# vitoplantamura/OnnxStream

Hardware: NVIDIA H100
Metric: SD1.5 UNet 512x512 bs=1 denoise steps/s (one UNet Model::run per step) (higher is better)
Workload: dtype f16

## Files before the change

### onnxstream_b200/csrc/attention_wgmma.cu

```cuda

#include "common.cuh"
#include "tc_ptx.cuh"
#include <cuda.h>
#include <cstdio>

namespace {

using namespace tcptx;

constexpr int BQ = 128;
constexpr int BKV = 128;
constexpr int KV_STAGES = 4;
constexpr int FA_THREADS = 384;
constexpr int FA_CONSUMERS = 256;
constexpr int FA_PRODUCER_REGS = 40, FA_CONSUMER_REGS = 232;

template <int NCH, int BK, int QKS, int KS = KV_STAGES, int PLANES = 1>
struct FaCfg {
    static_assert(QKS <= 4 * NCH && (BK == 32 || BK == 64 || BK == 128), "tile");
    static constexpr int Q_CHUNK = BQ * 128;
    static constexpr int KV_CHUNK = BK * 128;
    static constexpr int Q_PLANE = NCH * Q_CHUNK;
    static constexpr int KV_PLANE = NCH * KV_CHUNK;
    static constexpr int Q_BYTES = PLANES * Q_PLANE;
// ... 33 lines not shown
    return smem;
}

template <int KS, typename Load>
__device__ __forceinline__ void fa_produce_kv(uint64_t* kv_full, uint64_t* kv_empty, int n_kv, uint32_t tile_bytes, Load load)
{
    for (int j = 0; j < n_kv; j++) {
        const int st = j % KS;
        mbar_wait(&kv_empty[st], ((j / KS) & 1) ^ 1);
        if (elect_one()) {
            mbar_expect_tx(&kv_full[st], tile_bytes);
            load(st, j, &kv_full[st]);
        }
        __syncwarp();
    }
    osb_pdl_trigger_late();
}

template <int BK>
__device__ __forceinline__ float fa_row_max(const float (&s)[BK / 2], int h)
{
    float mt = -INFINITY;
#pragma unroll
    for (int c = 0; c < BK / 8; c++) mt = fmaxf(mt, fmaxf(s[4 * c + 2 * h], s[4 * c + 2 * h + 1]));
    mt = fmaxf(mt, __shfl_xor_sync(0xffffffffu, mt, 1));
    mt = fmaxf(mt, __shfl_xor_sync(0xffffffffu, mt, 2));
    return mt;
}

__device__ __forceinline__ float ex2_approx(float x)
{
// ... 110 lines not shown
#pragma unroll
            for (int h = 0; h < 2; h++) { o[ch][4 * c + 2 * h] *= alpha[h]; o[ch][4 * c + 2 * h + 1] *= alpha[h]; }
#pragma unroll
    for (int c = 0; c < BK / 8; c++)
#pragma unroll
        for (int h = 0; h < 2; h++) a[c >> 1][(c & 1) * 2 + h] = pack_half2(s[4 * c + 2 * h], s[4 * c + 2 * h + 1]);
}

template <int NCH, int BK, int QKS>
__global__ void __launch_bounds__(FA_THREADS, 1)
flash_attention_kernel(const __grid_constant__ CUtensorMap map_q, const __grid_constant__ CUtensorMap map_k, const __grid_constant__ CUtensorMap map_v,
                       const FaParams p)
{
    using C = FaCfg<NCH, BK, QKS>;
    constexpr int S = KV_STAGES;
    osb_pdl_trigger_entry();
    const int warp = threadIdx.x >> 5, lane = threadIdx.x & 31;
    const int head = blockIdx.y;
    const int q0 = blockIdx.x * BQ;
    const int n_kv = p.kv_tiles;
    uint8_t* smem = fa_prologue(&map_q, &map_k, &map_v, C::BARS, FA_CONSUMERS / 32, S);
    uint8_t* sQ = smem;
    uint8_t* sK = sQ + C::Q_BYTES;
    uint8_t* sV = sK + S * C::KV_BYTES;
    uint64_t* q_full = (uint64_t*)(smem + C::BARS);
    uint64_t* kv_full = q_full + 1;
    uint64_t* kv_empty = kv_full + S;

    if (warp < 4) {
        setmaxnreg_dec<FA_PRODUCER_REGS>();
        if (warp == 0) {
// ... 100 lines not shown
    const unsigned short* m = reinterpret_cast<const unsigned short*>(row) + col;
    if (col + 1 < Tk) {
        if (vec) return __ldg(reinterpret_cast<const unsigned int*>(m));
        return (uint32_t)__ldg(m) | ((uint32_t)__ldg(m + 1) << 16);
    }
    return col < Tk ? (uint32_t)__ldg(m) : 0u;
}

template <int NCH, int BK>
__global__ void __launch_bounds__(FA_THREADS, 1)
sdpa_flash_kernel(const __grid_constant__ CUtensorMap map_q, const __grid_constant__ CUtensorMap map_k, const __grid_constant__ CUtensorMap map_v,
                  const SdpaParams p)
{
    using C = FaCfg<NCH, BK, 4 * NCH>;
    constexpr float LOG2E = 1.4426950408889634f;
    osb_pdl_trigger_entry();
    const int warp = threadIdx.x >> 5, lane = threadIdx.x & 31;
    const int r0 = blockIdx.x * BQ, hk = blockIdx.y;
    const int n_kv = p.kv_tiles;
    uint8_t* smem = fa_prologue(&map_q, &map_k, &map_v, C::BARS, FA_CONSUMERS, KV_STAGES);
    uint8_t* sQ = smem;
    uint8_t* sK = sQ + C::Q_BYTES;
    uint8_t* sV = sK + KV_STAGES * C::KV_BYTES;
    uint64_t* q_full = (uint64_t*)(smem + C::BARS);
    uint64_t* kv_full = q_full + 1;
    uint64_t* kv_empty = kv_full + KV_STAGES;

    if (warp == 0) {
        if (elect_one()) {
            mbar_expect_tx(q_full, C::Q_BYTES);
#pragma unroll
// ... 152 lines not shown
    wgmma_fence();
#pragma unroll
    for (int kk = 0; kk < WD_BK / 16; kk++)
#pragma unroll
        for (int ch = 0; ch < WD_NV; ch++)
            wgmma_m64n64k16_f16_rs(o[ch], a[kk], vdesc + (uint64_t)((ch * WD_V_CHUNK + kk * 2048) >> 4), 1u);
    wgmma_commit();
}

template <bool KT>
__global__ void __launch_bounds__(WD_THREADS, 1)
flash_attention_wide_kernel(const __grid_constant__ CUtensorMap map_q, const __grid_constant__ CUtensorMap map_k,
                            const __grid_constant__ CUtensorMap map_v, const FaParams p)
{
    constexpr int KS = WD_K_STAGES, VS = WD_V_STAGES;
    osb_pdl_trigger_entry();
    const int warp = threadIdx.x >> 5, lane = threadIdx.x & 31;
    const int n_slices = (p.d + 64 * WD_NV - 1) / (64 * WD_NV);
    const int col0 = (blockIdx.x % n_slices) * (64 * WD_NV);
    const int q0 = (blockIdx.x / n_slices) * WD_BQ;
    const int head = blockIdx.y;
    const int n_dch = (p.d + 63) >> 6;
    uint8_t* smem = fa_prologue(&map_q, &map_k, &map_v, WD_BARS, WD_CONSUMERS / 32, KS, VS);
    uint8_t* sQ = smem;
    uint8_t* sK = sQ + WD_DCH * WD_Q_CHUNK;
    uint8_t* sV = sK + KS * WD_K_CHUNK;
    uint64_t* q_full = (uint64_t*)(smem + WD_BARS);
    uint64_t* k_full = q_full + 1;
    uint64_t* k_empty = k_full + KS;
    uint64_t* v_full = k_empty + KS;
    uint64_t* v_empty = v_full + VS;
// ... 17 lines not shown
                        mbar_expect_tx(&k_full[st], WD_K_CHUNK);
                        if (KT) tma_load_3d(sK + st * WD_K_CHUNK, &map_k, &k_full[st], j * WD_BK, 64 * c, head);
                        else tma_load_3d(sK + st * WD_K_CHUNK, &map_k, &k_full[st], 64 * c, j * WD_BK, head);
                    }
                    __syncwarp();
                }
                const int sv = j % VS;
                mbar_wait(&v_empty[sv], ((j / VS) & 1) ^ 1);
                if (elect_one()) {
                    mbar_expect_tx(&v_full[sv], n_vch * WD_V_CHUNK);
                    for (int ch = 0; ch < n_vch; ch++)
                        tma_load_3d(sV + sv * WD_V_BYTES + ch * WD_V_CHUNK, &map_v, &v_full[sv], col0 + 64 * ch, j * WD_BK, head);
                }
                __syncwarp();
            }
            osb_pdl_trigger_late();
        }
    } else {
        setmaxnreg_inc<WD_CONSUMER_REGS>();
        const int r = (warp & 3) * 16 + (lane >> 2);
        const int cq = 2 * (lane & 3);
        const uint64_t qdesc0 = make_smem_desc(smem_u32(sQ), 16, 1024);
        const uint64_t kdesc0 = make_smem_desc(smem_u32(sK), KT ? WD_K_CHUNK : 16, 1024);
        const uint64_t vdesc0 = make_smem_desc(smem_u32(sV), WD_V_CHUNK, 1024);
        float o[WD_NV][32];
#pragma unroll
        for (int ch = 0; ch < WD_NV; ch++)
#pragma unroll
            for (int i = 0; i < 32; i++) o[ch][i] = 0.f;
        float s[WD_BK / 2];
        uint32_t a[WD_BK / 16][4];
// ... 134 lines not shown
}

template <int BK>
__device__ __forceinline__ void qk_mma_bf16(float (&s)[BK / 2], uint64_t da, uint64_t db, uint32_t scale_d)
{
    if constexpr (BK == 64) wgmma_m64n64k16_bf16<0>(s, da, db, scale_d);
    else wgmma_m64n32k16_bf16<0>(s, da, db, scale_d);
}

template <int NCH, int BK, int QKS, int KS>
__global__ void __launch_bounds__(FA_THREADS, 1)
flash_attention_f32x_kernel(const __grid_constant__ CUtensorMap map_q, const __grid_constant__ CUtensorMap map_k, const __grid_constant__ CUtensorMap map_v,
                            const FaParams p, float scale, float* __restrict__ out)
{
    using C = FaCfg<NCH, BK, QKS, KS, 3>;
    osb_pdl_trigger_entry();
    const int warp = threadIdx.x >> 5, lane = threadIdx.x & 31;
    const int head = blockIdx.y, heads = gridDim.y;
    const int q0 = blockIdx.x * BQ;
    const int n_kv = p.kv_tiles;
    uint8_t* smem = fa_prologue(&map_q, &map_k, &map_v, C::BARS, FA_CONSUMERS / 32, KS);
    uint8_t* sQ = smem;
    uint8_t* sK = sQ + C::Q_BYTES;
    uint8_t* sV = sK + KS * C::KV_BYTES;
    uint64_t* q_full = (uint64_t*)(smem + C::BARS);
    uint64_t* kv_full = q_full + 1;
    uint64_t* kv_empty = kv_full + KS;

    if (warp < 4) {
        setmaxnreg_dec<FA_PRODUCER_REGS>();
        if (warp == 0) {
// ... 172 lines not shown
            __nv_bfloat16 h, m, l;
            bf16x3_split(tile[tx][i], h, m, l);
            const int64_t o = (int64_t)key * d + c;
            dst[o] = h;
            dst[(int64_t)Tk * d + o] = m;
            dst[2 * (int64_t)Tk * d + o] = l;
        }
    }
}

__global__ void __launch_bounds__(WD_THREADS, 1)
flash_attention_wide_f32x_kernel(const __grid_constant__ CUtensorMap map_q, const __grid_constant__ CUtensorMap map_k,
                                 const __grid_constant__ CUtensorMap map_v, const FaParams p, float scale, float* __restrict__ out)
{
    constexpr int QS = WX_QK_STAGES, VS = WX_V_STAGES;
    osb_pdl_trigger_entry();
    const int warp = threadIdx.x >> 5, lane = threadIdx.x & 31;
    const int n_slices = (p.d + 64 * WD_NV - 1) / (64 * WD_NV);
    const int col0 = (blockIdx.x % n_slices) * (64 * WD_NV);
    const int q0 = (blockIdx.x / n_slices) * WD_BQ;
    const int head = blockIdx.y;
    const int n_dch = (p.d + 63) >> 6;
    const int n_vch = min(WD_NV, (p.d - col0 + 63) >> 6);
    uint8_t* smem = fa_prologue(&map_q, &map_k, &map_v, WX_BARS, WD_CONSUMERS / 32, QS, VS);
    uint8_t* sQK = smem;
    uint8_t* sV = sQK + QS * WX_QK_BYTES;
    uint64_t* qk_full = (uint64_t*)(smem + WX_BARS) + 1;
    uint64_t* qk_empty = qk_full + QS;
    uint64_t* v_full = qk_empty + QS;
    uint64_t* v_empty = v_full + VS;
    const int n_kv = p.kv_tiles;
// ... 15 lines not shown
                        }
                    }
                    __syncwarp();
                }
                const int sv = j % VS;
                mbar_wait(&v_empty[sv], ((j / VS) & 1) ^ 1);
                if (elect_one()) {
                    mbar_expect_tx(&v_full[sv], 3 * n_vch * WX_V_CHUNK);
                    for (int pl = 0; pl < 3; pl++)
                        for (int ch = 0; ch < n_vch; ch++)
                            tma_load_3d(sV + sv * WX_V_BYTES + pl * WX_V_PLANE + ch * WX_V_CHUNK, &map_v, &v_full[sv], pl * p.d + col0 + 64 * ch,
                                        j * WX_BK, head);
                }
                __syncwarp();
            }
            osb_pdl_trigger_late();
        }
    } else {
        setmaxnreg_inc<WD_CONSUMER_REGS>();
        const int r = (warp & 3) * 16 + (lane >> 2);
        const int cq = 2 * (lane & 3);
        const uint64_t qdesc0 = make_smem_desc(smem_u32(sQK), 16, 1024);
        const uint64_t vdesc0 = make_smem_desc(smem_u32(sV), WX_V_CHUNK, 1024);
        float o[WD_NV][32];
#pragma unroll
        for (int ch = 0; ch < WD_NV; ch++)
#pragma unroll
            for (int i = 0; i < 32; i++) o[ch][i] = 0.f;
        float m_run[2] = { -INFINITY, -INFINITY }, l_run[2] = { 0.f, 0.f }, alpha[2];
        int kc = 0;
        for (int j = 0; j < n_kv; j++) {
// ... 122 lines not shown
__device__ __forceinline__ float2 ld_mask_pair_f32(const float* row, int col, int Tk, bool vec)
{
    if (col + 1 < Tk) {
        if (vec) return __ldg(reinterpret_cast<const float2*>(row + col));
        return make_float2(__ldg(row + col), __ldg(row + col + 1));
    }
    return make_float2(col < Tk ? __ldg(row + col) : 0.f, 0.f);
}

template <int NCH, int BK, int QKS, int KS>
__global__ void __launch_bounds__(FA_THREADS, 1)
sdpa_flash_f32x_kernel(const __grid_constant__ CUtensorMap map_q, const __grid_constant__ CUtensorMap map_k, const __grid_constant__ CUtensorMap map_v,
                       const SdpaF32xParams p)
{
    using C = FaCfg<NCH, BK, QKS, KS, 3>;
    osb_pdl_trigger_entry();
    const int warp = threadIdx.x >> 5, lane = threadIdx.x & 31;
    const int r0 = blockIdx.x * BQ, hk = blockIdx.y;
    const int n_kv = p.kv_tiles;
    uint8_t* smem = fa_prologue(&map_q, &map_k, &map_v, C::BARS, FA_CONSUMERS / 32, KS);
    uint8_t* sQ = smem;
    uint8_t* sK = sQ + C::Q_BYTES;
    uint8_t* sV = sK + KS * C::KV_BYTES;
    uint64_t* q_full = (uint64_t*)(smem + C::BARS);
    uint64_t* kv_full = q_full + 1;
    uint64_t* kv_empty = kv_full + KS;

    if (warp < 4) {
        setmaxnreg_dec<FA_PRODUCER_REGS>();
        if (warp == 0) {
            if (elect_one()) {
// ... 285 lines not shown
```

### onnxstream_b200/csrc/capi.cpp

```cpp
#include "engine_impl.h"
#include "plan.h"
#include "../../include/onnxstream_b200.h"

#include <cuda_profiler_api.h>
#include <cstdio>
#include <cstdlib>
#include <cstring>
#include <stdexcept>

using namespace osb;

struct ModelContext {
    std::unique_ptr<Engine> engine;
    std::string def;
    std::string wp;
    std::vector<std::string> upcast_patterns;
    Engine& E()
    {
        if (!engine) throw std::runtime_error("onnxstream_b200: this model was created without a backend (threads_count < 0)");
        return *engine;
    }
};

static char* dup_cstr(const std::string& s)
// ... 228 lines not shown
{
    std::string r;
    try {
        r = osb::plan_summary(model_text ? model_text : "", fp16_arithmetic != 0, fuse_nodes != 0, fuse_attention != 0, use_scaled_dp_attn_op != 0);
    } catch (const std::exception& e) {
        r = std::string("=== ERROR === ") + e.what();
    }
    char* buf = (char*)malloc(r.size() + 1);
    if (buf) memcpy(buf, r.c_str(), r.size() + 1);
    return buf;
}

int model_b200_get_stats(ModelContext* obj, double* out, int n)
{
    const EngineStats& s = obj->E().stats();
    double v[] = { (double)s.weight_ring_bytes, (double)s.weight_peak_live_bytes, (double)s.weight_largest_node_bytes,
                   (double)s.weight_bytes_streamed, (double)s.weight_resident_bytes, (double)s.act_high_water_bytes,
                   (double)s.h2d_input_bytes, (double)s.d2h_output_bytes, (double)s.kernel_launches, (double)s.tc_launches,
                   (double)s.ops_executed, (double)s.ops_fused_away, s.last_run_ms, s.last_gpu_ms, (double)s.graph_replays, (double)s.side_steps };
    int m = (int)(sizeof(v) / sizeof(v[0]));
    for (int i = 0; i < n && i < m; i++) out[i] = v[i];
    return m;
}

double model_b200_run_resident(ModelContext* obj, int steps)
{
    try { return obj->E().run_resident(steps); }
    catch (const std::exception& e) { fprintf(stderr, "=== ERROR === %s\n", e.what()); return -1.0; }
}

int model_b200_set_comm(ModelContext* obj, void* nccl_comm, int rank, int nranks)
{
    obj->E().set_comm((ncclComm*)nccl_comm, rank, nranks);
    return 0;
// ... 11 lines not shown
```

### onnxstream_b200/csrc/common.cuh

```cuda
#pragma once

#include <cuda_runtime.h>
#include <cuda_fp16.h>
#include <cuda_bf16.h>
#include <stdint.h>
#include <algorithm>
#include <utility>
#include "../../include/onnxstream_b200_kernels.h"

using std::min;
using std::max;

extern "C" void osb_count_launch(int tensor_core);

static inline int launched(int tensor_core = 0)
{
    osb_count_launch(tensor_core);
    return (int)cudaGetLastError();
}

__device__ __forceinline__ void osb_pdl_trigger() { asm volatile("griddepcontrol.launch_dependents;" ::: "memory"); }
__device__ __forceinline__ void osb_pdl_wait() { asm volatile("griddepcontrol.wait;" ::: "memory"); }
#ifdef OSB_PDL_LATE
__device__ __forceinline__ void osb_pdl_trigger_entry() {}
__device__ __forceinline__ void osb_pdl_trigger_late() { osb_pdl_trigger(); }
#else
__device__ __forceinline__ void osb_pdl_trigger_entry() { osb_pdl_trigger(); }
__device__ __forceinline__ void osb_pdl_trigger_late() {}
#endif
__device__ __forceinline__ void osb_pdl_prologue() { osb_pdl_trigger_entry(); osb_pdl_wait(); }

extern "C" int osb_pdl_enabled(void);

template <typename... KArgs, typename... Args>
static inline void osb_launch_cluster(void (*kernel)(KArgs...), dim3 grid, dim3 block, size_t smem, cudaStream_t st, unsigned cluster, Args&&... args)
{
    cudaLaunchConfig_t cfg{};
    cfg.gridDim = grid; cfg.blockDim = block; cfg.dynamicSmemBytes = smem; cfg.stream = st;
    cudaLaunchAttribute attr[2];
    int n = 0;
    if (osb_pdl_enabled()) {
        attr[n].id = cudaLaunchAttributeProgrammaticStreamSerialization;
        attr[n].val.programmaticStreamSerializationAllowed = 1;
        n++;
    }
// ... 118 lines not shown
```

### onnxstream_b200/csrc/engine.h

```cpp
#pragma once

#include <cstdint>
#include <cstddef>
#include <functional>
#include <map>
#include <memory>
#include <set>
#include <string>
#include <unordered_map>
#include <vector>

struct CUstream_st;
struct CUevent_st;
struct ncclComm;

namespace osb {

enum class DType : int { none = 0, u8 = 1, f16 = 2, f32 = 3, i64 = 4 };
enum class Layout : int { plain = 0, nhwc = 1 };

size_t dtype_size(DType t);
const char* dtype_name(DType t);

class DevicePool;
// ... 81 lines not shown

struct EngineStats {
    size_t weight_ring_bytes = 0;
    size_t weight_peak_live_bytes = 0;
    size_t weight_largest_node_bytes = 0;
    size_t weight_bytes_streamed = 0;
    size_t weight_resident_bytes = 0;
    size_t act_high_water_bytes = 0;
    size_t h2d_input_bytes = 0, d2h_output_bytes = 0;
    uint64_t kernel_launches = 0, tc_launches = 0;
    uint64_t ops_executed = 0, ops_fused_away = 0;
    double last_run_ms = 0.0;
    double last_gpu_ms = 0.0;
    int graph_replays = 0;
    int side_steps = 0;
};

struct PinnedBuf {
    void* ptr = nullptr;
    size_t bytes = 0;
    explicit PinnedBuf(size_t n);
    ~PinnedBuf();
};

struct HostTensor {
    std::string name;
    DType type = DType::none;
    std::vector<size_t> shape;
    std::shared_ptr<PinnedBuf> buf;
    size_t count = 0;
// ... 47 lines not shown
    bool is_model_empty() const { return m_text.empty(); }
    std::vector<std::pair<DType, std::string>> weights_names();

    void* push_input(const std::string& name, DType type, const std::vector<size_t>& shape);
    void run();
    double run_resident(int steps);
    std::vector<HostTensor>& tensors() { return m_host_tensors; }
    void clear_tensors();

    void read_range_data(const char* filename);
    void write_range_data(const char* filename);

    void set_comm(ncclComm* comm, int rank, int nranks);

    const EngineStats& stats() const { return m_stats; }
    int device() const { return m_device; }
    CUstream_st* compute_stream() const { return m_stream; }

private:
    int m_device = 0;
    CUstream_st* m_stream = nullptr;
    std::string m_text, m_path;
    std::vector<OpDef> m_ops;
    bool m_parsed = false;
    std::map<std::string, int> m_refs_initial;
    bool m_first_run = true;

    std::unique_ptr<WeightSource> m_source;
    std::unique_ptr<WeightStreamer> m_streamer;
    DevicePool m_pool;
// ... 20 lines not shown
```

### onnxstream_b200/csrc/engine_run.cpp

```cpp
#include "engine_impl.h"
#include "plan.h"
#include "workspace.h"

#include <limits>
#include <cuda_fp16.h>

#include <algorithm>
#include <chrono>
#include <cmath>
#include <cstdio>
#include <cstring>
#include <stdexcept>
#include <thread>
#include <tuple>

namespace osb {

namespace {

inline int K(DType t) { return (int)t; }

std::vector<int64_t> parse_ints(const std::string& s)
{
    std::vector<int64_t> v;
// ... 30 lines not shown
        if (side_stream) { cudaStreamSynchronize(side_stream); osb_workspace_release(side_stream); cudaStreamDestroy(side_stream); }
    }

    std::unordered_map<std::string, std::vector<Tensor>> store;
    std::vector<std::string> order;
    std::map<std::string, int> refs;

    Plan plan;
    std::string plan_signature;
    size_t next_stage = 0;
    std::map<std::pair<size_t, size_t>, std::pair<WeightStreamer::Slot*, size_t>> staged;
    std::map<size_t, WeightStreamer::Slot*> step_slot;

    std::unordered_map<std::string, Tensor> resident;
    size_t resident_bytes = 0;

    cudaStream_t side_stream = nullptr;
    DevicePool side_pool;
    bool on_side = false;
    std::vector<cudaEvent_t> side_events;
    DevicePool& pool() { return on_side ? side_pool : E.m_pool; }
    struct MhaKV { Tensor kl, vl; cudaEvent_t ev = nullptr; };
    std::map<size_t, MhaKV> mha_kv;
    void mha_project(size_t i, const Tensor& x, const Tensor* xq, Tensor* ql, Tensor& kl, Tensor& vl, int64_t Tka);
    void mha_prepass(size_t si);
    bool mha_flash(int64_t T, int64_t Tk, int64_t d, DType ty, float scale) const
    {
        if (!flash_on() || !(scale > 0.f && scale < INFINITY)) return false;
        return ty == DType::f32 ? osb_flash_attention_f32x_ok(T, Tk, d, K(ty)) : osb_flash_attention_ok(T, Tk, d, K(ty));
    }
// ... 2358 lines not shown
}

struct GraphState {
    cudaGraph_t graph = nullptr;
    cudaGraphExec_t exec = nullptr;
    struct In { std::string name; std::vector<size_t> shape; DevPtr dev; size_t bytes; DType type; };
    struct Out { std::string name; std::vector<size_t> shape; DevPtr dev; size_t count; DType type; };
    std::vector<In> inputs;
    std::vector<Out> outputs;
    std::vector<DevPtr> keepalive;
    bool ready = false;
    bool failed = false;
};
static std::map<Engine*, GraphState> g_graphs;

void Engine::drop_graph()
{
    auto it = g_graphs.find(this);
    if (it == g_graphs.end()) return;
    if (it->second.exec) cudaGraphExecDestroy(it->second.exec);
    if (it->second.graph) cudaGraphDestroy(it->second.graph);
    g_graphs.erase(it);
}

bool Engine::try_replay()
{
    auto it = g_graphs.find(this);
    if (it == g_graphs.end() || !it->second.ready) return false;
    GraphState& G = it->second;
    std::vector<HostTensor*> fins;
// ... 144 lines not shown
        }
        n_fresh = uploaded.size();
        for (auto& k : I.kept_inputs) uploaded.emplace_back(k, false);
    }
    std::vector<HostTensor> pinned_inputs = std::move(m_host_tensors);
    m_host_tensors.clear();

    bool capture_open = false;
    std::vector<std::tuple<std::string, std::vector<size_t>, Tensor>> finals;
    try {
        if (capturing) {
            check_cuda(cudaStreamSynchronize(m_stream), "pre-capture sync");
            check_cuda(cudaStreamBeginCapture(m_stream, cudaStreamCaptureModeRelaxed), "cudaStreamBeginCapture");
            capture_open = true;
        }
        for (size_t ui = 0; ui < uploaded.size(); ui++) {
            auto& u = uploaded[ui];
            Tensor t = u.first;
            if (ui >= n_fresh) {  }
            else if ((use_uint8_qdq || use_uint8_arithmetic) && (t.type == DType::f32 || t.type == DType::f16)) { t = I.quantize_dynamic(t); t.name = u.first.name; }
            else if (u.second) { t = I.convert(t, DType::f16); t.name = u.first.name; }
            if (keep_inputs && ui < n_fresh && t.type != DType::i64) I.kept_inputs.push_back(t);
            auto& v = I.store[t.name];
            if (v.empty()) I.order.push_back(t.name);
            v.push_back(std::move(t));
        }
        if (!I.gn_ring) I.gn_ring = m_pool.alloc(2048);
        check_cuda(cudaMemsetAsync(I.gn_ring->ptr, 0, 2048, m_stream), "cudaMemsetAsync(gn ring)");
        I.gn_slot = 0; I.gn_slot_used[0] = I.gn_slot_used[1] = 0; I.stats_ready_for = -1; I.stats_want = -1;
        I.mha_kv.clear();
        bool hoist = !I.plan.is_side.empty() && resident_weights && !m_first_run && !has_i64_input && !ops_times_printf && !ops_printf && m_nranks == 1;
        if (hoist) { std::set<std::string> seen; for (auto& u : uploaded) if (!seen.insert(u.first.name).second) hoist = false; }
        m_stats.side_steps = 0;
        if (hoist) {
            for (size_t si = 0; si < I.plan.steps.size(); si++) m_stats.side_steps += (I.plan.is_side[si] || (!I.plan.kv_side.empty() && I.plan.kv_side[si])) ? 1 : 0;
            if (!I.side_stream) check_cuda(cudaStreamCreateWithFlags(&I.side_stream, cudaStreamNonBlocking), "cudaStreamCreate(side)");
            if (I.side_events.size() != I.plan.steps.size() + 2) {
                for (auto e : I.side_events) if (e) cudaEventDestroy(e);
                I.side_events.assign(I.plan.steps.size() + 2, nullptr);
            }
            auto ev = [&](size_t k) -> cudaEvent_t& { if (!I.side_events[k]) check_cuda(cudaEventCreateWithFlags(&I.side_events[k], cudaEventDisableTiming), "cudaEventCreate"); return I.side_events[k]; };
            const size_t EV_IN = I.plan.steps.size(), EV_DONE = I.plan.steps.size() + 1;
            check_cuda(cudaEventRecord(ev(EV_IN), m_stream), "cudaEventRecord(inputs)");
// ... 44 lines not shown
                t = I.convert(t, DType::f32);
                if (t.dev.get() == t0_.dev.get() && capturing) {
                    Tensor c = I.make(DType::f32, t.shape);
                    check_cuda(cudaMemcpyAsync(c.mdata(), t.data(), (size_t)t.numel() * 4, cudaMemcpyDeviceToDevice, m_stream), "copy");
                    t = c;
                }
                finals.emplace_back(name, shp, t);
            }
        }
        if (capturing) {
            if (I.capture_unsafe) throw std::runtime_error("an op read the values of an int64 graph input on the host: not capturable");
            for (auto& f : finals) if (std::get<2>(f).type == DType::i64) throw std::runtime_error("int64 graph outputs are host-evaluated: not capturable");
            capture_open = false;
            check_cuda(cudaStreamEndCapture(m_stream, &G->graph), "cudaStreamEndCapture");
            check_cuda(cudaGraphInstantiate(&G->exec, G->graph, 0), "cudaGraphInstantiate");
            for (auto& f : finals) if (std::get<2>(f).type != DType::i64) G->outputs.push_back({ std::get<0>(f), std::get<1>(f), std::get<2>(f).dev, (size_t)std::get<2>(f).numel(), std::get<2>(f).type });
            check_cuda(cudaGraphLaunch(G->exec, m_stream), "cudaGraphLaunch");
            G->ready = true;
            m_pool.frozen = false;
        }
    } catch (...) {
        if (capture_open) { cudaGraph_t junk = nullptr; cudaStreamEndCapture(m_stream, &junk); if (junk) cudaGraphDestroy(junk); }
        if (capturing) { auto& g = g_graphs[this]; g.failed = true; g.inputs.clear(); g.outputs.clear(); }
        I.store.clear(); I.order.clear(); I.silu_cache.clear();
        cudaEventDestroy(ev0); cudaEventDestroy(ev1);
        if (capturing) {
            cudaGetLastError();
            m_host_tensors = std::move(pinned_inputs);
            use_cuda_graph = false;
            run();
// ... 56 lines not shown
```

### onnxstream_b200/csrc/gemm_i8.cuh

```cuda

namespace i8k {

constexpr int I8_BLOCK_K = 128;
constexpr int I8_WG_K = 32;
constexpr int I8_STAGES = 4;
constexpr int I8_STAGE_BYTES = A_STAGE_BYTES + 2 * B_STAGE_BYTES;
constexpr int I8_SMEM = I8_STAGES * I8_STAGE_BYTES + 1024 + 256;
constexpr int TRANSPOSE_THREADS = 96;

struct I8Params {
    int M, N, K;
    int m_tiles, n_tiles;
    int b_kmajor;
    int taps, kw, Wo, Ho, bw, bh, tiles_x, k_blocks_per_tap, stride;
    int Wp;
    const int32_t* rsum;
    const int32_t* csum;
    const int32_t* bias;
    int zx, zw, zy;
    int kzz;
    float requant;
    uint8_t* C;
    long long ldc;
};

__global__ void __launch_bounds__(NUM_THREADS, 1)
tc_i8_kernel(const __grid_constant__ CUtensorMap map_a, const __grid_constant__ CUtensorMap map_b, const I8Params p)
{
    osb_pdl_trigger_entry();
    extern __shared__ uint8_t smem_raw[];
    uint8_t* smem = (uint8_t*)(((uintptr_t)smem_raw + 1023) & ~(uintptr_t)1023);
    uint8_t* smem_a = smem;
    uint8_t* smem_b = smem + I8_STAGES * A_STAGE_BYTES;
    uint8_t* smem_stg = smem_b + I8_STAGES * B_STAGE_BYTES;
    uint64_t* bars = (uint64_t*)(smem + I8_STAGES * I8_STAGE_BYTES);
    uint64_t* full = bars;
    uint64_t* empty = bars + I8_STAGES;
    uint64_t* stg_full = empty + I8_STAGES;

    const int warp = threadIdx.x >> 5, lane = threadIdx.x & 31;
    if (warp == 0 && lane == 0) {
        asm volatile("prefetch.tensormap [%0];" ::"l"(&map_a) : "memory");
        asm volatile("prefetch.tensormap [%0];" ::"l"(&map_b) : "memory");
    }
// ... 31 lines not shown
                        mbar_expect_tx(&full[stage], A_STAGE_BYTES + B_STAGE_BYTES);
                        tma_load_3d_s(sb0 + stage * B_STAGE_BYTES, &map_b, &full[stage], kglob, n0, 0);
                    } else {
                        mbar_expect_tx(&full[stage], A_STAGE_BYTES);
                        mbar_expect_tx(&stg_full[stage], B_STAGE_BYTES);
                        tma_load_3d_s(sg0 + stage * B_STAGE_BYTES, &map_b, &stg_full[stage], n0, kglob, 0);
                    }
                    if (p.bh > 0) tma_load_3d_s(sa, &map_a, &full[stage], kc, ax + kx, ay + ky);
                    else tma_load_3d_s(sa, &map_a, &full[stage], kc, m0, 0);
                }
                __syncwarp();
                if (++kcb == p.k_blocks_per_tap) { kcb = 0; tap++; if (++kx == p.kw) { kx = 0; ky++; } }
                if (++stage == I8_STAGES) { stage = 0; phase ^= 1; }
            }
        }
        osb_pdl_trigger_late();
    } else if (warp < 4) {
        if (p.b_kmajor) return;
        const int t = (int)threadIdx.x - 32;
        int stage = 0; uint32_t phase = 0;
        for (int tile = blockIdx.x; tile < total_tiles; tile += gridDim.x) {
            for (int kb = 0; kb < k_blocks; kb++) {
                mbar_wait(&stg_full[stage], phase);
                const uint8_t* stg = smem_stg + stage * B_STAGE_BYTES;
                uint8_t* dst = smem_b + stage * B_STAGE_BYTES;
                for (int n = t; n < BLOCK_N; n += TRANSPOSE_THREADS) {
#pragma unroll
                    for (int c = 0; c < I8_BLOCK_K / 16; c++) {
                        uint32_t w[4];
#pragma unroll
                        for (int q = 0; q < 4; q++) {
// ... 151 lines not shown
```

### onnxstream_b200/csrc/gemm_wgmma.cu

```cuda

#include "common.cuh"
#include "workspace.h"
#include "tc_ptx.cuh"
#include <cuda.h>
#include <cstdio>
#include <cstdlib>
#include <vector>

namespace {

constexpr int BLOCK_M = 128;
constexpr int BLOCK_N = 128;
constexpr int BLOCK_K = 64;
constexpr int WG_K = 16;
constexpr int RING_BYTES = 6 * 32768;
constexpr int NUM_THREADS = 384;
constexpr int CONSUMER_THREADS = 256;

template <int BM, int BN>
struct TileCfg {
    static constexpr int A_STAGE_BYTES = BM * BLOCK_K * 2;
    static constexpr int B_STAGE_BYTES = BN * BLOCK_K * 2;
    static constexpr int STAGES_FIT = RING_BYTES / (A_STAGE_BYTES + B_STAGE_BYTES);
    static constexpr int STAGES = STAGES_FIT < 16 ? STAGES_FIT : 16;
// ... 58 lines not shown
    else v = (ok0 ? (uint32_t)(NC ? __ldg(s) : s[0]) : 0u) | (ok1 ? (uint32_t)(NC ? __ldg(s + 1) : s[1]) << 16 : 0u);
    return *reinterpret_cast<__half2*>(&v);
}


template <int BM, int BN, bool EXTRAS, int B_MN_MAJOR, bool BF16, bool PAIR, bool GEGLU = false>
__global__ void __launch_bounds__(NUM_THREADS, 1)
tc_gemm_kernel(const __grid_constant__ CUtensorMap map_a, const __grid_constant__ CUtensorMap map_b, const __grid_constant__ CUtensorMap map_b1,
               const __grid_constant__ CUtensorMap map_b2, const TcParams p)
{
    using Cfg = TileCfg<BM, BN>;
    constexpr int STAGES = Cfg::STAGES, A_STAGE_BYTES = Cfg::A_STAGE_BYTES, B_STAGE_BYTES = Cfg::B_STAGE_BYTES, WN = Cfg::WN;
    static_assert(!PAIR || (BM == 128 && BN == 128), "CTA pairs run 128 x 128 tiles");
    static_assert(!B_MN_MAJOR || WN % 64 == 0, "an MN-major B is read in 64-column atoms");
    static_assert(!GEGLU || (BM == 128 && BN == 128 && B_MN_MAJOR && !EXTRAS && !BF16 && !PAIR), "GEGLU: 128 x 128 tiles of an fp16 [K, 2 N] weight");
    osb_pdl_trigger_entry();
    extern __shared__ uint8_t smem_raw[];
    uint8_t* smem = (uint8_t*)(((uintptr_t)smem_raw + 1023) & ~(uintptr_t)1023);
    uint8_t* smem_a = smem;
    uint8_t* smem_b = smem + STAGES * A_STAGE_BYTES;
    uint64_t* bars = (uint64_t*)(smem + STAGES * (A_STAGE_BYTES + B_STAGE_BYTES));
    uint64_t* full = bars;
    uint64_t* empty = bars + STAGES;
    double* gn_acc = (double*)((uint8_t*)bars + 256);

    const int warp = threadIdx.x >> 5;
    const int lane = threadIdx.x & 31;
    if (EXTRAS && p.gn_stats && threadIdx.x < 2 * GN_MAX_GROUPS) gn_acc[threadIdx.x] = 0.0;

    if (warp == 0 && lane == 0) {
        asm volatile("prefetch.tensormap [%0];" ::"l"(&map_a) : "memory");
// ... 59 lines not shown
                        else tma_load_3d_s(sb, mbp, &full[stage], kglob, n0, b);
                    } else {
#pragma unroll
                        for (int at = 0; at < BN / 64; at++) {
                            const int col = GEGLU ? 64 * nt + at * p.N : n0 + 64 * at;
                            if (p.b_swap) tma_load_3d_s(sb + at * 8192, mbp, &full[stage], col, b, kglob);
                            else tma_load_3d_s(sb + at * 8192, mbp, &full[stage], col, kglob, b);
                        }
                    }
                }
                __syncwarp();
                if (++kcb == p.k_blocks_per_tap) { kcb = 0; tap++; if (++kx == p.kw) { kx = 0; ky++; } }
                if (++stage == STAGES) { stage = 0; phase ^= 1; }
            }
        }
        osb_pdl_trigger_late();
    } else if (warp >= 4) {
        const int wg = (warp >> 2) - 1;
        const int ct = (int)threadIdx.x - (NUM_THREADS - CONSUMER_THREADS);
        const int wrow = BM == 128 ? 64 * wg : 0, wcol = BM == 128 ? 0 : WN * wg;
        const uint64_t adesc0 = make_smem_desc(smem_u32(smem_a) + wrow * 128, 16, 1024);
        const uint64_t bdesc0 = B_MN_MAJOR ? make_smem_desc(smem_u32(smem_b) + (wcol / 64) * 8192, 8192, 1024) : make_smem_desc(smem_u32(smem_b) + wcol * 128, 16, 1024);
        const bool partial = p.split_k > 1 || p.f32_out;
        const int r_lo = wrow + (warp & 3) * 16 + (lane >> 2);
        const int cq = 2 * (lane & 3);
        const bool vec_bias = ((uintptr_t)p.bias & 3) == 0, vec_bias2 = ((uintptr_t)p.bias2 & 3) == 0;
        const bool vec_res = ((uintptr_t)p.residual & 3) == 0 && ((p.ldc | p.stride_c) & 1) == 0;
        auto release = [&](int s) {
            if (PAIR) {
                __syncwarp();
                if (lane == 0) { mbar_arrive(&empty[s]); mbar_arrive_remote(&empty[s], rank ^ 1u); }
// ... 234 lines not shown

__device__ __forceinline__ void f16x2_bf16_parts(uint32_t v, uint32_t& hi, uint32_t& lo)
{
    const float2 x = __half22float2(*reinterpret_cast<const __half2*>(&v));
    const __nv_bfloat162 h = __float22bfloat162_rn(x);
    const float2 hf = __bfloat1622float2(h);
    const __nv_bfloat162 l = __float22bfloat162_rn(make_float2(x.x - hf.x, x.y - hf.y));
    hi = *reinterpret_cast<const uint32_t*>(&h);
    lo = *reinterpret_cast<const uint32_t*>(&l);
}

__global__ void __launch_bounds__(NUM_THREADS, 1)
tc_gemm_f16w_kernel(const __grid_constant__ CUtensorMap map_a, const __grid_constant__ CUtensorMap map_b, const TcParams p)
{
    using namespace f16w;
    osb_pdl_trigger_entry();
    extern __shared__ uint8_t smem_raw[];
    uint8_t* smem = (uint8_t*)(((uintptr_t)smem_raw + 1023) & ~(uintptr_t)1023);
    uint8_t* smem_a = smem;
    uint8_t* smem_b = smem + STAGES * A_BYTES;
    uint64_t* bars = (uint64_t*)(smem + STAGES * (A_BYTES + B_BYTES));
    uint64_t* full = bars;
    uint64_t* empty = bars + STAGES;
    uint64_t* landed = bars + 2 * STAGES;
    const int warp = threadIdx.x >> 5, lane = threadIdx.x & 31;
    if (warp == 0 && lane == 0) {
        asm volatile("prefetch.tensormap [%0];" ::"l"(&map_a) : "memory");
        asm volatile("prefetch.tensormap [%0];" ::"l"(&map_b) : "memory");
    }
    if (warp == 1 && lane == 0) {
        for (int i = 0; i < STAGES; i++) { mbar_init(&full[i], 3); mbar_init(&empty[i], CONSUMER_THREADS); mbar_init(&landed[i], 1); }
// ... 17 lines not shown
            for (int kb = kb_lo; kb < kb_hi; kb++) {
                mbar_wait(&empty[stage], phase ^ 1);
                if (elect_one()) {
                    mbar_expect_tx(&landed[stage], A_BYTES + B_PART_BYTES);
                    const int kc = kb * BLOCK_K;
                    const uint32_t sa = sa0 + stage * A_BYTES, sb = sb0 + stage * B_BYTES;
#pragma unroll
                    for (int pl = 0; pl < 3; pl++) tma_load_3d_s(sa + pl * A_PLANE_BYTES, &map_a, &landed[stage], pl * p.K + kc, m0, 0);
#pragma unroll
                    for (int at = 0; at < 2; at++) tma_load_3d_s(sb + at * 8192, &map_b, &landed[stage], n0 + 64 * at, kc, 0);
                }
                __syncwarp();
                if (++stage == STAGES) { stage = 0; phase ^= 1; }
            }
        }
        osb_pdl_trigger_late();
    } else if (warp < 4) {
        const int t = (int)threadIdx.x - 32;
        constexpr int PER = (B_PART_BYTES / 16 + SPLIT_THREADS - 1) / SPLIT_THREADS;
        int stage = 0; uint32_t phase = 0;
        for (int tile = blockIdx.x; tile < total; tile += gridDim.x) {
            const int sp = tile % p.split_k;
            const int kb_lo = sp * kb_per_split, kb_hi = min(kb_lo + kb_per_split, kbk);
            for (int kb = kb_lo; kb < kb_hi; kb++) {
                mbar_wait(&landed[stage], phase);
                uint4* bh = reinterpret_cast<uint4*>(smem_b + stage * B_BYTES);
                uint4* bl = reinterpret_cast<uint4*>(smem_b + stage * B_BYTES + B_PART_BYTES);
                uint4 v[PER];
#pragma unroll
                for (int j = 0; j < PER; j++) if (t + j * SPLIT_THREADS < B_PART_BYTES / 16) v[j] = bh[t + j * SPLIT_THREADS];
#pragma unroll
// ... 731 lines not shown
```

### onnxstream_b200/csrc/kernels_basic.cu

```cuda

#include "common.cuh"
#include <cuda_bf16.h>
#include <cstring>
#include "workspace.h"
#include <cstdio>
#include <cstdlib>

namespace {


template <typename S, typename D>
__global__ void convert_kernel(const S* __restrict__ src, D* __restrict__ dst, size_t n)
{
    osb_pdl_prologue();
    for (size_t i = blockIdx.x * (size_t)blockDim.x + threadIdx.x; i < n; i += (size_t)gridDim.x * blockDim.x)
        dst[i] = from_float<D>(to_float(src[i]));
}

template <typename D>
__global__ void dequant_kernel(const uint8_t* __restrict__ src, D* __restrict__ dst, size_t n, float scale, int zp)
{
    osb_pdl_prologue();
    for (size_t i = blockIdx.x * (size_t)blockDim.x + threadIdx.x; i < n; i += (size_t)gridDim.x * blockDim.x)
        dst[i] = from_float<D>((float)((int)src[i] - zp) * scale);
// ... 711 lines not shown
            unsigned cum = 0, d = 0;
            for (; d < 256; d++) { if (cum + hist[d] > rank) break; cum += hist[d]; }
            bcast[0] = d; bcast[1] = rank - cum;
        }
        __syncthreads();
        prefix |= bcast[0] << shift; mask |= 255u << shift; rank = bcast[1];
        __syncthreads();
    }
    return prefix;
}

template <typename T>
__global__ void __launch_bounds__(1024, 1)
percentile_chunks_kernel(const T* __restrict__ x, size_t size, size_t threads, size_t chunk, float from_left, float from_right, unsigned* __restrict__ out)
{
    extern __shared__ unsigned pk[];
    __shared__ unsigned hist[256], bcast[2], n_finite;
    size_t per = size / threads; if (!per) per = 1;
    const size_t i = blockIdx.y;
    const size_t start = i * per, end = i >= threads - 1 ? size : (i + 1) * per;
    if (start >= end || start >= size) return;
    const size_t c0 = start + (size_t)blockIdx.x * chunk;
    if (c0 >= end) return;
    const int n = (int)min(chunk, end - c0);
    constexpr bool half = sizeof(T) == 2;
    if (threadIdx.x == 0) n_finite = 0;
    __syncthreads();
    unsigned local = 0;
    for (int j = threadIdx.x; j < n; j += blockDim.x) {
        unsigned key;
// ... 592 lines not shown
    if (n == 0) return 0;
    if (dtype != OSB_F16 && dtype != OSB_F32) return (int)cudaErrorInvalidValue;
    if (threads < 1) threads = 1;
    const size_t chunk = dtype == OSB_F16 ? 32768 : 16384;
    size_t per = n / (size_t)threads; if (!per) per = 1;
    const size_t longest = std::max(per, n - per * ((size_t)threads - 1 < n / per ? (size_t)threads - 1 : n / per));
    dim3 grid((unsigned)((longest + chunk - 1) / chunk), (unsigned)threads);
    const size_t smem = chunk * sizeof(unsigned);
    static bool attr = false;
    if (!attr) {
        cudaFuncSetAttribute(percentile_chunks_kernel<__half>, cudaFuncAttributeMaxDynamicSharedMemorySize, (int)(32768 * 4));
        cudaFuncSetAttribute(percentile_chunks_kernel<float>, cudaFuncAttributeMaxDynamicSharedMemorySize, (int)(16384 * 4));
        attr = true;
    }
    cudaStream_t st = (cudaStream_t)stream;
    if (dtype == OSB_F16) percentile_chunks_kernel<__half><<<grid, 1024, smem, st>>>((const __half*)x, n, (size_t)threads, chunk, from_left, from_right, (unsigned*)out3);
    else percentile_chunks_kernel<float><<<grid, 1024, smem, st>>>((const float*)x, n, (size_t)threads, chunk, from_left, from_right, (unsigned*)out3);
    return launched();
}

float osb_percentile_key_to_float(unsigned key, int dtype)
{
    if (dtype == OSB_F16) {
        unsigned short h = (key & 0x8000u) ? (unsigned short)(key & 0x7FFFu) : (unsigned short)(~key & 0xFFFFu);
        __half hv; memcpy(&hv, &h, 2);
        return __half2float(hv);
    }
    unsigned u = (key & 0x80000000u) ? (key & 0x7FFFFFFFu) : ~key;
    float f; memcpy(&f, &u, 4);
    return f;
}

// ... 107 lines not shown
```

### onnxstream_b200/csrc/kernels_gemm.cu

```cuda

#include "common.cuh"
#include "workspace.h"
#include <cstdlib>

int osb_tc_gemm_launch(const void* A, const void* B, void* C, const void* bias, const void* residual,
                       int64_t batch, int64_t M, int64_t N, int64_t K, int64_t sa, int64_t sb, int64_t sc,
                       int b_transposed, cudaStream_t st, int64_t lda, int64_t ldb, int64_t ldc);
int osb_tc_conv_launch(const void* x, const void* w, const void* bias, const void* residual, void* y,
                       int64_t H, int64_t W, int64_t Cin, int64_t Cout, int kh, int kw, int stride, int pad_top, int pad_left,
                       int64_t Ho, int64_t Wo, cudaStream_t st, const void* bias2, double* gn_stats, int gn_groups, int* gn_done);
int osb_tc_gemm_grouped_launch(const void* A, const void* const* B, void* const* C, int groups, int64_t M, int64_t N, int64_t K, int bt, cudaStream_t st,
                               int64_t lda, int64_t ldb, int64_t ldc);
bool osb_tc_gemm_ok(int64_t M, int64_t N, int64_t K, int b_transposed, const void* A, const void* B, const void* C, int64_t sa, int64_t sb, int64_t sc,
                    int64_t lda, int64_t ldb, int64_t ldc);
bool osb_tc_conv_ok(int64_t H, int64_t W, int64_t Cin, int64_t Cout, int kh, int kw, int stride, const void* x, const void* w, const void* y);

namespace {

struct ConvGeom {
    int H, W, Cin, kh, kw, stride, pad_top, pad_left, Ho, Wo;
};

constexpr int BM = 64, BN = 64, BK = 16;

// ... 925 lines not shown
        }
    }
    int warps = 4;
    size_t smem = (size_t)warps * (d + dv + 32) * sizeof(float);
    if (smem > 48 * 1024) return (int)cudaErrorInvalidValue;
    int grid = (int)min<int64_t>((heads * Tq + warps - 1) / warps, OSB_SMS * 8);
    if (dtype == OSB_F16) osb_launch((attention_rows_kernel<__half>), grid, warps * 32, smem, st, (const __half*)q, (const __half*)k, (const __half*)v, (const __half*)mask, (__half*)out, heads, Tq, Tk, (int)d, (int)dv, scale, k_transposed, kv_group);
    else if (dtype == OSB_F32) osb_launch((attention_rows_kernel<float>), grid, warps * 32, smem, st, (const float*)q, (const float*)k, (const float*)v, (const float*)mask, (float*)out, heads, Tq, Tk, (int)d, (int)dv, scale, k_transposed, kv_group);
    else return (int)cudaErrorInvalidValue;
    return launched();
}

static int g_pdl = -1;
int osb_pdl_enabled(void)
{
    if (g_pdl < 0) { const char* e = getenv("OSB_PDL"); g_pdl = (e && e[0] == '1') ? 1 : 0; }
    return g_pdl;
}
void osb_set_pdl(int enable) { g_pdl = enable ? 1 : 0; }
static uint64_t g_launches = 0, g_tc_launches = 0;
void osb_count_launch(int tensor_core) { g_launches++; if (tensor_core) g_tc_launches++; }
uint64_t osb_launch_count(void) { return g_launches; }
uint64_t osb_tc_launch_count(void) { return g_tc_launches; }
void osb_launch_count_reset(void) { g_launches = 0; g_tc_launches = 0; }

}
```

### onnxstream_b200/model.py

```python
from __future__ import annotations

import ctypes
import os
import re
from typing import Dict, List, Optional, Sequence, Tuple

import numpy as np

_PKG_DIR = os.path.dirname(os.path.abspath(__file__))
ENGINE_LIB = os.environ.get("OSB_ENGINE_LIB") or os.path.join(_PKG_DIR, "csrc", "libonnxstream_b200.so")

OPTION_NAMES = (
    "use_fp16_arithmetic", "use_uint8_qdq", "use_uint8_arithmetic", "fuse_ops_in_attention",
    "force_fp16_storage", "support_dynamic_shapes", "use_ops_cache", "use_scaled_dp_attn_op",
    "use_next_op_cache", "ops_printf", "ops_times_printf", "use_nchw_convs",
)


class OnnxStreamError(RuntimeError):
    pass


class _TensorView(ctypes.Structure):
    _fields_ = [("dims_num", ctypes.c_size_t), ("dims", ctypes.POINTER(ctypes.c_size_t)),
# ... 173 lines not shown
    def add_upcast_pattern(self, pattern: str):
        self.lib.model_ext_add_upcast_pattern(self.h, pattern.encode())

    def get_tensor_i64(self, name: str) -> Optional[np.ndarray]:
        cap = 1 << 20
        buf = (ctypes.c_longlong * cap)()
        dims = (ctypes.c_size_t * 8)()
        nd = ctypes.c_size_t(0)
        n = self.lib.model_ext_get_tensor_i64(self.h, name.encode(), buf, cap, dims, ctypes.byref(nd))
        if n < 0:
            return None
        return np.array(buf[:n], dtype=np.int64).reshape(tuple(dims[i] for i in range(nd.value)))

    STAT_FIELDS = ("weight_ring_bytes", "weight_peak_live_bytes", "weight_largest_node_bytes", "weight_bytes_streamed",
                   "weight_resident_bytes", "act_high_water_bytes", "h2d_input_bytes", "d2h_output_bytes", "kernel_launches",
                   "tc_launches", "steps_executed", "ops_fused_away", "last_run_ms", "last_gpu_ms", "graph_replays", "side_steps")

    def run_resident(self, steps: int) -> float:
        ms = self.lib.model_b200_run_resident(self.h, steps)
        if ms < 0:
            raise OnnxStreamError("model_b200_run_resident failed (no captured graph?)")
        return ms

    def stats(self) -> Dict[str, float]:
        out = (ctypes.c_double * len(self.STAT_FIELDS))()
        self.lib.model_b200_get_stats(self.h, out, len(self.STAT_FIELDS))
        return dict(zip(self.STAT_FIELDS, list(out)))
```

Measured before the change: 197.3.

## Enable programmatic dependent launch by default with late triggers after producer loops

Turns PDL on by default: the OSB_PDL env variable now has to be set to 0 to disable it, where before it had to be set to 1 to enable it. The launch_dependents trigger moves from kernel entry to the end of the producer loads in the attention and GEMM kernels, and to after the wait in the generic prologue. It also routes percentile_chunks through osb_launch with a PDL prologue, and moves the gn-ring memset ahead of the uploads so kernels sit next to each other in the captured graph. The goal is to overlap each kernel's launch and prologue with the tail of the previous kernel inside the CUDA graph. It also adds a graph census of nodes and programmatic edges to the stats. The risk is added griddepcontrol waits and ordering hazards if any kernel reads its predecessor's outputs before waiting.

```diff
diff --git a/onnxstream_b200/csrc/attention_wgmma.cu b/onnxstream_b200/csrc/attention_wgmma.cu
--- a/onnxstream_b200/csrc/attention_wgmma.cu
+++ b/onnxstream_b200/csrc/attention_wgmma.cu
@@ -71,7 +71,7 @@
         }
         __syncwarp();
     }
-    osb_pdl_trigger_late();
+    osb_pdl_trigger();
 }
 
 template <int BK>
@@ -212,7 +212,6 @@
 {
     using C = FaCfg<NCH, BK, QKS>;
     constexpr int S = KV_STAGES;
-    osb_pdl_trigger_entry();
     const int warp = threadIdx.x >> 5, lane = threadIdx.x & 31;
     const int head = blockIdx.y;
     const int q0 = blockIdx.x * BQ;
@@ -343,7 +342,6 @@
 {
     using C = FaCfg<NCH, BK, 4 * NCH>;
     constexpr float LOG2E = 1.4426950408889634f;
-    osb_pdl_trigger_entry();
     const int warp = threadIdx.x >> 5, lane = threadIdx.x & 31;
     const int r0 = blockIdx.x * BQ, hk = blockIdx.y;
     const int n_kv = p.kv_tiles;
@@ -526,7 +524,6 @@
                             const __grid_constant__ CUtensorMap map_v, const FaParams p)
 {
     constexpr int KS = WD_K_STAGES, VS = WD_V_STAGES;
-    osb_pdl_trigger_entry();
     const int warp = threadIdx.x >> 5, lane = threadIdx.x & 31;
     const int n_slices = (p.d + 64 * WD_NV - 1) / (64 * WD_NV);
     const int col0 = (blockIdx.x % n_slices) * (64 * WD_NV);
@@ -574,7 +571,7 @@
                 }
                 __syncwarp();
             }
-            osb_pdl_trigger_late();
+            osb_pdl_trigger();
         }
     } else {
         setmaxnreg_inc<WD_CONSUMER_REGS>();
@@ -739,7 +736,6 @@
                             const FaParams p, float scale, float* __restrict__ out)
 {
     using C = FaCfg<NCH, BK, QKS, KS, 3>;
-    osb_pdl_trigger_entry();
     const int warp = threadIdx.x >> 5, lane = threadIdx.x & 31;
     const int head = blockIdx.y, heads = gridDim.y;
     const int q0 = blockIdx.x * BQ;
@@ -942,7 +938,6 @@
                                  const __grid_constant__ CUtensorMap map_v, const FaParams p, float scale, float* __restrict__ out)
 {
     constexpr int QS = WX_QK_STAGES, VS = WX_V_STAGES;
-    osb_pdl_trigger_entry();
     const int warp = threadIdx.x >> 5, lane = threadIdx.x & 31;
     const int n_slices = (p.d + 64 * WD_NV - 1) / (64 * WD_NV);
     const int col0 = (blockIdx.x % n_slices) * (64 * WD_NV);
@@ -988,7 +983,7 @@
                 }
                 __syncwarp();
             }
-            osb_pdl_trigger_late();
+            osb_pdl_trigger();
         }
     } else {
         setmaxnreg_inc<WD_CONSUMER_REGS>();
@@ -1141,7 +1136,6 @@
                        const SdpaF32xParams p)
 {
     using C = FaCfg<NCH, BK, QKS, KS, 3>;
-    osb_pdl_trigger_entry();
     const int warp = threadIdx.x >> 5, lane = threadIdx.x & 31;
     const int r0 = blockIdx.x * BQ, hk = blockIdx.y;
     const int n_kv = p.kv_tiles;
diff --git a/onnxstream_b200/csrc/capi.cpp b/onnxstream_b200/csrc/capi.cpp
--- a/onnxstream_b200/csrc/capi.cpp
+++ b/onnxstream_b200/csrc/capi.cpp
@@ -266,10 +266,12 @@
 int model_b200_get_stats(ModelContext* obj, double* out, int n)
 {
     const EngineStats& s = obj->E().stats();
+    const GraphCensus g = obj->E().graph_census();
     double v[] = { (double)s.weight_ring_bytes, (double)s.weight_peak_live_bytes, (double)s.weight_largest_node_bytes,
                    (double)s.weight_bytes_streamed, (double)s.weight_resident_bytes, (double)s.act_high_water_bytes,
                    (double)s.h2d_input_bytes, (double)s.d2h_output_bytes, (double)s.kernel_launches, (double)s.tc_launches,
-                   (double)s.ops_executed, (double)s.ops_fused_away, s.last_run_ms, s.last_gpu_ms, (double)s.graph_replays, (double)s.side_steps };
+                   (double)s.ops_executed, (double)s.ops_fused_away, s.last_run_ms, s.last_gpu_ms, (double)s.graph_replays, (double)s.side_steps,
+                   (double)g.kernel_nodes, (double)g.other_nodes, (double)g.kernel_edges, (double)g.programmatic_edges };
     int m = (int)(sizeof(v) / sizeof(v[0]));
     for (int i = 0; i < n && i < m; i++) out[i] = v[i];
     return m;
diff --git a/onnxstream_b200/csrc/common.cuh b/onnxstream_b200/csrc/common.cuh
--- a/onnxstream_b200/csrc/common.cuh
+++ b/onnxstream_b200/csrc/common.cuh
@@ -21,14 +21,7 @@
 
 __device__ __forceinline__ void osb_pdl_trigger() { asm volatile("griddepcontrol.launch_dependents;" ::: "memory"); }
 __device__ __forceinline__ void osb_pdl_wait() { asm volatile("griddepcontrol.wait;" ::: "memory"); }
-#ifdef OSB_PDL_LATE
-__device__ __forceinline__ void osb_pdl_trigger_entry() {}
-__device__ __forceinline__ void osb_pdl_trigger_late() { osb_pdl_trigger(); }
-#else
-__device__ __forceinline__ void osb_pdl_trigger_entry() { osb_pdl_trigger(); }
-__device__ __forceinline__ void osb_pdl_trigger_late() {}
-#endif
-__device__ __forceinline__ void osb_pdl_prologue() { osb_pdl_trigger_entry(); osb_pdl_wait(); }
+__device__ __forceinline__ void osb_pdl_prologue() { osb_pdl_wait(); osb_pdl_trigger(); }
 
 extern "C" int osb_pdl_enabled(void);
 
diff --git a/onnxstream_b200/csrc/engine.h b/onnxstream_b200/csrc/engine.h
--- a/onnxstream_b200/csrc/engine.h
+++ b/onnxstream_b200/csrc/engine.h
@@ -119,6 +119,10 @@
     double last_gpu_ms = 0.0;
     int graph_replays = 0;
     int side_steps = 0;
+};
+
+struct GraphCensus {
+    int kernel_nodes = 0, other_nodes = 0, kernel_edges = 0, programmatic_edges = 0;
 };
 
 struct PinnedBuf {
@@ -196,6 +200,7 @@
     void set_comm(ncclComm* comm, int rank, int nranks);
 
     const EngineStats& stats() const { return m_stats; }
+    GraphCensus graph_census() const;
     int device() const { return m_device; }
     CUstream_st* compute_stream() const { return m_stream; }
 
diff --git a/onnxstream_b200/csrc/engine_run.cpp b/onnxstream_b200/csrc/engine_run.cpp
--- a/onnxstream_b200/csrc/engine_run.cpp
+++ b/onnxstream_b200/csrc/engine_run.cpp
@@ -68,6 +68,7 @@
 
     std::unordered_map<std::string, Tensor> resident;
     size_t resident_bytes = 0;
+    GraphCensus census;
 
     cudaStream_t side_stream = nullptr;
     DevicePool side_pool;
@@ -2456,6 +2457,34 @@
 };
 static std::map<Engine*, GraphState> g_graphs;
 
+static void count_graph(cudaGraph_t g, GraphCensus& s)
+{
+    size_t n = 0, ne = 0;
+    check_cuda(cudaGraphGetNodes(g, nullptr, &n), "cudaGraphGetNodes");
+    std::vector<cudaGraphNode_t> nodes(n);
+    check_cuda(cudaGraphGetNodes(g, nodes.data(), &n), "cudaGraphGetNodes");
+    std::set<cudaGraphNode_t> kernels;
+    for (auto nd : nodes) {
+        cudaGraphNodeType t;
+        check_cuda(cudaGraphNodeGetType(nd, &t), "cudaGraphNodeGetType");
+        if (t == cudaGraphNodeTypeKernel) kernels.insert(nd);
+    }
+    check_cuda(cudaGraphGetEdges_v2(g, nullptr, nullptr, nullptr, &ne), "cudaGraphGetEdges_v2");
+    std::vector<cudaGraphNode_t> from(ne), to(ne);
+    std::vector<cudaGraphEdgeData> data(ne);
+    check_cuda(cudaGraphGetEdges_v2(g, from.data(), to.data(), data.data(), &ne), "cudaGraphGetEdges_v2");
+    s = GraphCensus{};
+    s.kernel_nodes = (int)kernels.size();
+    s.other_nodes = (int)(n - kernels.size());
+    for (size_t e = 0; e < ne; e++) {
+        if (!kernels.count(from[e]) || !kernels.count(to[e])) continue;
+        s.kernel_edges++;
+        if (data[e].type == cudaGraphDependencyTypeProgrammatic) s.programmatic_edges++;
+    }
+}
+
+GraphCensus Engine::graph_census() const { return m_impl->census; }
+
 void Engine::drop_graph()
 {
     auto it = g_graphs.find(this);
@@ -2630,6 +2659,8 @@
             check_cuda(cudaStreamBeginCapture(m_stream, cudaStreamCaptureModeRelaxed), "cudaStreamBeginCapture");
             capture_open = true;
         }
+        if (!I.gn_ring) I.gn_ring = m_pool.alloc(2048);
+        check_cuda(cudaMemsetAsync(I.gn_ring->ptr, 0, 2048, m_stream), "cudaMemsetAsync(gn ring)");
         for (size_t ui = 0; ui < uploaded.size(); ui++) {
             auto& u = uploaded[ui];
             Tensor t = u.first;
@@ -2641,8 +2672,6 @@
             if (v.empty()) I.order.push_back(t.name);
             v.push_back(std::move(t));
         }
-        if (!I.gn_ring) I.gn_ring = m_pool.alloc(2048);
-        check_cuda(cudaMemsetAsync(I.gn_ring->ptr, 0, 2048, m_stream), "cudaMemsetAsync(gn ring)");
         I.gn_slot = 0; I.gn_slot_used[0] = I.gn_slot_used[1] = 0; I.stats_ready_for = -1; I.stats_want = -1;
         I.mha_kv.clear();
         bool hoist = !I.plan.is_side.empty() && resident_weights && !m_first_run && !has_i64_input && !ops_times_printf && !ops_printf && m_nranks == 1;
@@ -2717,6 +2746,7 @@
             capture_open = false;
             check_cuda(cudaStreamEndCapture(m_stream, &G->graph), "cudaStreamEndCapture");
             check_cuda(cudaGraphInstantiate(&G->exec, G->graph, 0), "cudaGraphInstantiate");
+            count_graph(G->graph, I.census);
             for (auto& f : finals) if (std::get<2>(f).type != DType::i64) G->outputs.push_back({ std::get<0>(f), std::get<1>(f), std::get<2>(f).dev, (size_t)std::get<2>(f).numel(), std::get<2>(f).type });
             check_cuda(cudaGraphLaunch(G->exec, m_stream), "cudaGraphLaunch");
             G->ready = true;
diff --git a/onnxstream_b200/csrc/gemm_i8.cuh b/onnxstream_b200/csrc/gemm_i8.cuh
--- a/onnxstream_b200/csrc/gemm_i8.cuh
+++ b/onnxstream_b200/csrc/gemm_i8.cuh
@@ -27,7 +27,6 @@
 __global__ void __launch_bounds__(NUM_THREADS, 1)
 tc_i8_kernel(const __grid_constant__ CUtensorMap map_a, const __grid_constant__ CUtensorMap map_b, const I8Params p)
 {
-    osb_pdl_trigger_entry();
     extern __shared__ uint8_t smem_raw[];
     uint8_t* smem = (uint8_t*)(((uintptr_t)smem_raw + 1023) & ~(uintptr_t)1023);
     uint8_t* smem_a = smem;
@@ -89,7 +88,7 @@
                 if (++stage == I8_STAGES) { stage = 0; phase ^= 1; }
             }
         }
-        osb_pdl_trigger_late();
+        osb_pdl_trigger();
     } else if (warp < 4) {
         if (p.b_kmajor) return;
         const int t = (int)threadIdx.x - 32;
diff --git a/onnxstream_b200/csrc/gemm_wgmma.cu b/onnxstream_b200/csrc/gemm_wgmma.cu
--- a/onnxstream_b200/csrc/gemm_wgmma.cu
+++ b/onnxstream_b200/csrc/gemm_wgmma.cu
@@ -96,7 +96,6 @@
     static_assert(!PAIR || (BM == 128 && BN == 128), "CTA pairs run 128 x 128 tiles");
     static_assert(!B_MN_MAJOR || WN % 64 == 0, "an MN-major B is read in 64-column atoms");
     static_assert(!GEGLU || (BM == 128 && BN == 128 && B_MN_MAJOR && !EXTRAS && !BF16 && !PAIR), "GEGLU: 128 x 128 tiles of an fp16 [K, 2 N] weight");
-    osb_pdl_trigger_entry();
     extern __shared__ uint8_t smem_raw[];
     uint8_t* smem = (uint8_t*)(((uintptr_t)smem_raw + 1023) & ~(uintptr_t)1023);
     uint8_t* smem_a = smem;
@@ -186,7 +185,7 @@
                 if (++stage == STAGES) { stage = 0; phase ^= 1; }
             }
         }
-        osb_pdl_trigger_late();
+        osb_pdl_trigger();
     } else if (warp >= 4) {
         const int wg = (warp >> 2) - 1;
         const int ct = (int)threadIdx.x - (NUM_THREADS - CONSUMER_THREADS);
@@ -451,7 +450,6 @@
 tc_gemm_f16w_kernel(const __grid_constant__ CUtensorMap map_a, const __grid_constant__ CUtensorMap map_b, const TcParams p)
 {
     using namespace f16w;
-    osb_pdl_trigger_entry();
     extern __shared__ uint8_t smem_raw[];
     uint8_t* smem = (uint8_t*)(((uintptr_t)smem_raw + 1023) & ~(uintptr_t)1023);
     uint8_t* smem_a = smem;
@@ -499,7 +497,7 @@
                 if (++stage == STAGES) { stage = 0; phase ^= 1; }
             }
         }
-        osb_pdl_trigger_late();
+        osb_pdl_trigger();
     } else if (warp < 4) {
         const int t = (int)threadIdx.x - 32;
         constexpr int PER = (B_PART_BYTES / 16 + SPLIT_THREADS - 1) / SPLIT_THREADS;
diff --git a/onnxstream_b200/csrc/kernels_basic.cu b/onnxstream_b200/csrc/kernels_basic.cu
--- a/onnxstream_b200/csrc/kernels_basic.cu
+++ b/onnxstream_b200/csrc/kernels_basic.cu
@@ -749,6 +749,7 @@
 __global__ void __launch_bounds__(1024, 1)
 percentile_chunks_kernel(const T* __restrict__ x, size_t size, size_t threads, size_t chunk, float from_left, float from_right, unsigned* __restrict__ out)
 {
+    osb_pdl_prologue();
     extern __shared__ unsigned pk[];
     __shared__ unsigned hist[256], bcast[2], n_finite;
     size_t per = size / threads; if (!per) per = 1;
@@ -1371,8 +1372,8 @@
         attr = true;
     }
     cudaStream_t st = (cudaStream_t)stream;
-    if (dtype == OSB_F16) percentile_chunks_kernel<__half><<<grid, 1024, smem, st>>>((const __half*)x, n, (size_t)threads, chunk, from_left, from_right, (unsigned*)out3);
-    else percentile_chunks_kernel<float><<<grid, 1024, smem, st>>>((const float*)x, n, (size_t)threads, chunk, from_left, from_right, (unsigned*)out3);
+    if (dtype == OSB_F16) osb_launch((percentile_chunks_kernel<__half>), grid, 1024, smem, st, (const __half*)x, n, (size_t)threads, chunk, from_left, from_right, (unsigned*)out3);
+    else osb_launch((percentile_chunks_kernel<float>), grid, 1024, smem, st, (const float*)x, n, (size_t)threads, chunk, from_left, from_right, (unsigned*)out3);
     return launched();
 }
 
diff --git a/onnxstream_b200/csrc/kernels_gemm.cu b/onnxstream_b200/csrc/kernels_gemm.cu
--- a/onnxstream_b200/csrc/kernels_gemm.cu
+++ b/onnxstream_b200/csrc/kernels_gemm.cu
@@ -963,7 +963,7 @@
 static int g_pdl = -1;
 int osb_pdl_enabled(void)
 {
-    if (g_pdl < 0) { const char* e = getenv("OSB_PDL"); g_pdl = (e && e[0] == '1') ? 1 : 0; }
+    if (g_pdl < 0) { const char* e = getenv("OSB_PDL"); g_pdl = (e && e[0] == '0') ? 0 : 1; }
     return g_pdl;
 }
 void osb_set_pdl(int enable) { g_pdl = enable ? 1 : 0; }
diff --git a/onnxstream_b200/model.py b/onnxstream_b200/model.py
--- a/onnxstream_b200/model.py
+++ b/onnxstream_b200/model.py
@@ -211,7 +211,8 @@
 
     STAT_FIELDS = ("weight_ring_bytes", "weight_peak_live_bytes", "weight_largest_node_bytes", "weight_bytes_streamed",
                    "weight_resident_bytes", "act_high_water_bytes", "h2d_input_bytes", "d2h_output_bytes", "kernel_launches",
-                   "tc_launches", "steps_executed", "ops_fused_away", "last_run_ms", "last_gpu_ms", "graph_replays", "side_steps")
+                   "tc_launches", "steps_executed", "ops_fused_away", "last_run_ms", "last_gpu_ms", "graph_replays", "side_steps",
+                   "graph_kernel_nodes", "graph_other_nodes", "graph_kernel_edges", "graph_programmatic_edges")
 
     def run_resident(self, steps: int) -> float:
         ms = self.lib.model_b200_run_resident(self.h, steps)
```

Result: faster. 202.4 (median of 6 runs) (+2.6%).
